# AtharvRN/dflash

Hardware: AMD Instinct MI355X
Metric: accepted_tokens_per_sec (higher is better)
Workload: dtype bf16

## Files before the change

### dflash_amd/csrc/attn_head.hip

```cpp
#include "gemm_rows.h"
#include <stdlib.h>
#include <type_traits>

namespace {

typedef __attribute__((address_space(3))) bf16x4 lds_bf16x4;

struct HeadAttnArgs {
  const bf16_t *xq;
  int64_t ldq;
  int q_col, k_col, v_col;
  const bf16_t *xc;
  int64_t ldc;
  int ck_col, cv_col;
  const bf16_t *q_w, *k_w;
  float eps;
  const bf16_t *cos_tab, *sin_tab;
  int max_pos;
  bf16_t *kc, *vc;
  int cache_rows;
  int n_q, n_kv, G;
  float scale_log2;
  int causal;
  const int32_t *dyn;
  int S, tau, bs, pos0;
  bf16x8 *out_frag;
  int64_t out_tile_stride;
  float *o_part;
  float *ml_part;
  int *tickets;
  int ns_old;
  int64_t xq_cand_stride, out_cand_stride, ws_cand_stride, cache_cand_stride;
  int dyn_cand_stride;
  const float *xq32;
  int64_t part_stride32;
  int nparts32;
  bf16_t *k_out, *v_out;
  int64_t kv_out_cand_stride;
  int out_rows;
};

__device__ __forceinline__ void swap16(float &a, float &b) {
  asm volatile("s_nop 1\n\tv_permlane16_swap_b32 %0, %1" : "+v"(a), "+v"(b));
}
__device__ __forceinline__ void swap32(float &a, float &b) {
  asm volatile("s_nop 1\n\tv_permlane32_swap_b32 %0, %1" : "+v"(a), "+v"(b));
}
__device__ __forceinline__ float wave_g_max(float v) {
  float a = v, b = v;
  swap16(a, b);
  a = b = fmaxf(a, b);
  swap32(a, b);
  return fmaxf(a, b);
}
__device__ __forceinline__ float wave_g_sum(float v) {
  float a = v, b = v;
  swap16(a, b);
  a = b = a + b;
  swap32(a, b);
  return a + b;
}

template <int NP>
struct RopeLoads {
  bf16x8 xv[NP], cs[NP], sn[NP], wv;
  f32x4 pa[NP][2], pb[NP][2];
};

template <int NP>
__device__ __forceinline__ void rope_issue(const bf16_t *const (&src)[NP], const int (&pos)[NP], const bf16_t *nw,
                                           const bf16_t *cos_tab, const bf16_t *sin_tab, int max_pos, const bf16_t *safe,
                                           int l, RopeLoads<NP> &ld) {
  const int d0 = (l & 15) * 8;
#pragma unroll
  for (int p = 0; p < NP; ++p) {
    ld.xv[p] = *reinterpret_cast<const bf16x8 *>((src[p] ? src[p] : safe) + d0);
    int pp = pos[p] < max_pos ? pos[p] : max_pos - 1;
    pp = pp < 0 ? 0 : pp;
    ld.cs[p] = *reinterpret_cast<const bf16x8 *>(cos_tab + (int64_t)pp * 64 + (d0 & 63));
    ld.sn[p] = *reinterpret_cast<const bf16x8 *>(sin_tab + (int64_t)pp * 64 + (d0 & 63));
  }
  ld.wv = *reinterpret_cast<const bf16x8 *>((nw ? nw : safe) + d0);
}

template <int NP>
__device__ __forceinline__ void rope_issue32(const float *const (&src)[NP], const int (&pos)[NP], const bf16_t *nw,
                                             const bf16_t *cos_tab, const bf16_t *sin_tab, int max_pos, const float *safe32,
                                             const bf16_t *safe, int64_t part_stride, int nparts, int l, RopeLoads<NP> &ld) {
  const int d0 = (l & 15) * 8;
  const int64_t ps = nparts > 1 ? part_stride : 0;
#pragma unroll
  for (int p = 0; p < NP; ++p) {
    const float *b = (src[p] ? src[p] : safe32) + d0;
    ld.pa[p][0] = *reinterpret_cast<const f32x4 *>(b);
    ld.pa[p][1] = *reinterpret_cast<const f32x4 *>(b + 4);
    ld.pb[p][0] = *reinterpret_cast<const f32x4 *>(b + ps);
    ld.pb[p][1] = *reinterpret_cast<const f32x4 *>(b + ps + 4);
    int pp = pos[p] < max_pos ? pos[p] : max_pos - 1;
    pp = pp < 0 ? 0 : pp;
    ld.cs[p] = *reinterpret_cast<const bf16x8 *>(cos_tab + (int64_t)pp * 64 + (d0 & 63));
    ld.sn[p] = *reinterpret_cast<const bf16x8 *>(sin_tab + (int64_t)pp * 64 + (d0 & 63));
  }
  ld.wv = *reinterpret_cast<const bf16x8 *>((nw ? nw : safe) + d0);
}
template <int NP>
__device__ __forceinline__ void rope_sum32(RopeLoads<NP> &ld, int nparts) {
#pragma unroll
  for (int p = 0; p < NP; ++p)
#pragma unroll
    for (int j = 0; j < 8; ++j) {
      const float s0 = ld.pa[p][j >> 2][j & 3], s1 = ld.pb[p][j >> 2][j & 3];
      ld.xv[p][j] = f2bf(nparts > 1 ? s0 + s1 : s0);
    }
}

template <int NP>
__device__ __forceinline__ void rope_finish(const RopeLoads<NP> &ld, const bool (&rope)[NP], bool has_norm, float eps, int l,
                                            bf16x8 (&out)[NP]) {
  const int c = l & 15;
#pragma unroll
  for (int p = 0; p < NP; ++p) {
    float x[8], n[8];
    float ss = 0.f;
#pragma unroll
    for (int j = 0; j < 8; ++j) {
      x[j] = bf2f(ld.xv[p][j]);
      ss += x[j] * x[j];
    }
    if (has_norm) {
      ss += __builtin_bit_cast(float, __builtin_amdgcn_mov_dpp(__builtin_bit_cast(int, ss), 0xB1, 0xF, 0xF, true));
      ss += __builtin_bit_cast(float, __builtin_amdgcn_mov_dpp(__builtin_bit_cast(int, ss), 0x4E, 0xF, 0xF, true));
      ss += __builtin_bit_cast(float, __builtin_amdgcn_mov_dpp(__builtin_bit_cast(int, ss), 0x141, 0xF, 0xF, true));
      ss += __builtin_bit_cast(float, __builtin_amdgcn_mov_dpp(__builtin_bit_cast(int, ss), 0x140, 0xF, 0xF, true));
      const float rstd = rsqrtf(ss * (1.f / 128.f) + eps);
#pragma unroll
      for (int j = 0; j < 8; ++j) n[j] = rbf(bf2f(ld.wv[j]) * rbf(x[j] * rstd));
    } else {
#pragma unroll
      for (int j = 0; j < 8; ++j) n[j] = x[j];
    }
#pragma unroll
    for (int j = 0; j < 8; ++j) {
      const float pn =
          __builtin_bit_cast(float, __builtin_amdgcn_mov_dpp(__builtin_bit_cast(int, n[j]), 0x128, 0xF, 0xF, true));
      const float cj = bf2f(ld.cs[p][j]), sj = bf2f(ld.sn[p][j]);
      const float r = rbf(rbf(n[j] * cj) + rbf((c < 8 ? -pn : pn) * sj));
      out[p][j] = f2bf(rope[p] ? r : x[j]);
    }
  }
}

template <int NP>
__device__ __forceinline__ void rope_items(const bf16_t *const (&src)[NP], const int (&pos)[NP], const bool (&rope)[NP],
                                           const bf16_t *nw, float eps, const bf16_t *cos_tab, const bf16_t *sin_tab,
                                           int max_pos, const bf16_t *safe, int l, bf16x8 (&out)[NP]) {
  RopeLoads<NP> ld;
  rope_issue<NP>(src, pos, nw, cos_tab, sin_tab, max_pos, safe, l, ld);
  rope_finish<NP>(ld, rope, nw != nullptr, eps, l, out);
}

__device__ __forceinline__ int k_swz(int row, int ch) { return row * 256 + ((ch ^ (row & 15)) << 4); }
__device__ __forceinline__ int v_swz(int row, int ch) {
  return row * 256 + ((((ch >> 1) ^ (row & 7)) << 5) | ((ch & 1) << 4));
}

#ifdef DFL_ATTN_STAMPS
__device__ unsigned long long g_hstamps[2][8];
#define HSTAMP(i)                                                                                  \
  do {                                                                                             \
    if (tid == 0 && kvh == 0 && hh == 0 && (split == 0 || is_new))                                 \
      g_hstamps[is_new ? 1 : 0][i] = __builtin_amdgcn_s_memrealtime();                             \
  } while (0)
__device__ unsigned long long g_ostamps[2][8];
__device__ unsigned long long g_amax[16];
#define OSTAMP(i)                                                                                  \
  do {                                                                                             \
    if (tid == 0 && (t == 0 || t == p.ntiles - 1)) g_ostamps[t ? 1 : 0][i] = __builtin_amdgcn_s_memrealtime(); \
  } while (0)
#else
#define HSTAMP(i)
#define OSTAMP(i)
#endif

template <int QT, int NW>
struct HeadLds {
  static_assert(NW * 4 >= QT * 16 && NW * 8192 >= 32768, "q rows: 4 per wave; new K / V: two 32-row tiles each");
  static constexpr int kVPriv = NW * 8192;
  static constexpr int kQ = kVPriv;
  static constexpr int kLoop = kVPriv + QT * 4096;
  static constexpr int kRow = 132;
  static constexpr int kMergeO = 0;
  static constexpr int kMergeML = NW * QT * 16 * kRow * 4;
  static constexpr int kMerge = kMergeML + NW * QT * 128;
  static constexpr int kRaw = kLoop > kMerge ? kLoop : kMerge;
  static constexpr int kBytes = NW < 8 ? kRaw : (kRaw > 84 * 1024 ? kRaw : 84 * 1024);
};

template <int QT, int NW, bool SIGNAL, bool HP = false, bool XF32 = false>
__device__ __forceinline__ void attn_head_body(const HeadAttnArgs &a, char *lds, int *s_last_p, const int kvh, const int by,
                                               const int cand, int *done_ctr) {
  static_assert(!HP || QT == 2, "head pairs use the two-tile register layout");
  using L = HeadLds<QT, NW>;
  int &s_last = *s_last_p;

  const int tid = threadIdx.x;
  const int w = __builtin_amdgcn_readfirstlane(tid >> 6), l = tid & 63;
  const int hpg = HP ? a.G >> 1 : a.G;
  const int hh = by % hpg, split = by / hpg;
  const int head = kvh * a.G + (HP ? 2 * hh : hh);
  const int ns = a.ns_old + 1;
  const bool is_new = split == a.ns_old;
  int S = a.S, tau = a.tau, bs = a.bs, pos0 = a.pos0;
  if (a.dyn) {
    const int32_t *dp = a.dyn + cand * a.dyn_cand_stride;
    S = dp[DFL_DYN_S];
    tau = dp[DFL_DYN_TAU];
    bs = dp[DFL_DYN_BS];
    pos0 = dp[DFL_DYN_POS0];
  }
  const int n_new = tau + bs;
  const int qi = l & 15, g = l >> 4;
  HSTAMP(0);
  const bf16_t *const xq = XF32 ? a.cos_tab : a.xq + cand * a.xq_cand_stride;
  const float *const xq32 = XF32 ? a.xq32 + cand * a.xq_cand_stride : nullptr;
  bf16x8 *const out_frag = a.out_frag + cand * a.out_cand_stride;
  float *const o_part = a.o_part + cand * a.ws_cand_stride;
  float *const ml_part = a.ml_part + cand * a.ws_cand_stride;
  int *const tickets = a.tickets + cand * a.ws_cand_stride;
  bf16_t *const kc = a.kc + cand * a.cache_cand_stride, *const vc = a.vc + cand * a.cache_cand_stride;
  bf16_t *const k_new = a.k_out ? a.k_out + cand * a.kv_out_cand_stride : kc;
  bf16_t *const v_new = a.k_out ? a.v_out + cand * a.kv_out_cand_stride : vc;
  const int new_rows_cap = a.k_out ? a.out_rows : a.cache_rows;
  const int new_row0 = a.k_out ? 0 : S;
  const bf16_t *kbase = kc + (int64_t)kvh * a.cache_rows * 128;
  const bf16_t *vbase = vc + (int64_t)kvh * a.cache_rows * 128;


  int t0 = 0, t1 = 0;
  if (!is_new && a.ns_old > 0) {
    const int nt = (S + 31) >> 5;
    const int tps = (nt + a.ns_old - 1) / a.ns_old;
    t0 = split * tps;
    t1 = t0 + tps;
    t0 = t0 > nt ? nt : t0;
    t1 = t1 > nt ? nt : t1;
  }
  const int old_last = S > 0 ? S - 1 : 0;
  bf16x8 kA[2][4], vA[8], kB[2][4], vB[8];
  auto fetch_k = [&](bf16x8(&kf)[2][4], int t, int lim) {
#pragma unroll
    for (int u = 0; u < 2; ++u) {
      int row = t * 32 + u * 16 + qi;
      row = row < lim ? row : lim;
#pragma unroll
      for (int s = 0; s < 4; ++s)
        kf[u][s] = *reinterpret_cast<const bf16x8 *>(kbase + (int64_t)row * 128 + s * 32 + g * 8);
    }
  };
  auto fetch_v = [&](bf16x8(&vr)[8], int t, int lim) {
#pragma unroll
    for (int i = 0; i < 8; ++i) {
      const int c = l + 64 * i;
      int row = t * 32 + (c >> 4);
      row = row < lim ? row : lim;
      vr[i] = *reinterpret_cast<const bf16x8 *>(vbase + (int64_t)row * 128 + (c & 15) * 8);
    }
  };
  auto fetch = [&](bf16x8(&kf)[2][4], bf16x8(&vr)[8], int t, int lim) {
    fetch_k(kf, t, lim);
    fetch_v(vr, t, lim);
  };
  char *q_lds = lds + L::kQ;
  const int jq = 4 * w + g;
  const int jrow = HP ? jq & 15 : jq;
  const int jhead = HP ? head + (jq >> 4) : head;
  RopeLoads<1> qld;
  {
    const int pos[1] = {pos0 + tau + jrow};
    if constexpr (XF32) {
      const float *src[1] = {jrow < bs ? xq32 + (int64_t)jrow * a.ldq + a.q_col + jhead * 128 : nullptr};
      rope_issue32<1>(src, pos, a.q_w, a.cos_tab, a.sin_tab, a.max_pos, xq32, xq, a.part_stride32, a.nparts32, l, qld);
    } else {
      const bf16_t *src[1] = {jrow < bs ? xq + (int64_t)jrow * a.ldq + a.q_col + jhead * 128 : nullptr};
      rope_issue<1>(src, pos, a.q_w, a.cos_tab, a.sin_tab, a.max_pos, xq, l, qld);
    }
  }
  asm volatile("" ::: "memory");
  auto finish_q = [&]() {
    if (jq < QT * 16) {
      const bool rp[1] = {true};
      bf16x8 ov[1];
      if constexpr (XF32) rope_sum32<1>(qld, a.nparts32);
      rope_finish<1>(qld, rp, a.q_w != nullptr, a.eps, l, ov);
      const bf16x8 z = {0, 0, 0, 0, 0, 0, 0, 0};
      *reinterpret_cast<bf16x8 *>(q_lds + (jq >> 4) * 4096 + k_swz(jq & 15, qi)) = jrow < bs ? ov[0] : z;
    }
  };
  int tcur = t0 + w;
  char *new_k = lds, *new_v = lds + 16384;
  if (!is_new) {
    fetch(kA, vA, tcur < t1 ? tcur : 0, old_last);
    asm volatile("" ::: "memory");
    finish_q();
  } else {
    auto sweep = [&](auto np_tag) {
      constexpr int NP = decltype(np_tag)::value;
      const bf16_t *src[NP];
      const float *src32[NP];
      int pos[NP], rel[NP];
      bool rp[NP], isv[NP];
      bf16x8 ov[NP];
#pragma unroll
      for (int p = 0; p < NP; ++p) {
        const int it = (p * NW + w) * 4 + g;
        isv[p] = it >= n_new;
        rel[p] = isv[p] ? it - n_new : it;
        const bool ok = it < 2 * n_new;
        const int vsel = isv[p] ? 1 : 0;
        if constexpr (XF32) {
          src32[p] = ok ? xq32 + (int64_t)rel[p] * a.ldq + a.k_col + vsel * (a.v_col - a.k_col) + kvh * 128 : nullptr;
          src[p] = ok ? xq : nullptr;
        } else {
          const bf16_t *row = rel[p] < tau ? a.xc + (int64_t)rel[p] * a.ldc + a.ck_col + vsel * (a.cv_col - a.ck_col)
                                           : xq + (int64_t)(rel[p] - tau) * a.ldq + a.k_col + vsel * (a.v_col - a.k_col);
          src[p] = ok ? row + kvh * 128 : nullptr;
          src32[p] = nullptr;
        }
        pos[p] = pos0 + rel[p];
        rp[p] = !isv[p];
      }
      RopeLoads<NP> kld;
      if constexpr (XF32)
        rope_issue32<NP>(src32, pos, a.k_w, a.cos_tab, a.sin_tab, a.max_pos, xq32, xq, a.part_stride32, a.nparts32, l, kld);
      else
        rope_issue<NP>(src, pos, a.k_w, a.cos_tab, a.sin_tab, a.max_pos, xq, l, kld);
      asm volatile("" ::: "memory");
      finish_q();
      if constexpr (XF32) rope_sum32<NP>(kld, a.nparts32);
      rope_finish<NP>(kld, rp, a.k_w != nullptr, a.eps, l, ov);
#pragma unroll
      for (int p = 0; p < NP; ++p)
        if (src[p]) {
          const int jt = rel[p] >> 5, r = rel[p] & 31;
          *reinterpret_cast<bf16x8 *>((isv[p] ? new_v + jt * 8192 + v_swz(r, qi) : new_k + jt * 8192 + k_swz(r, qi))) = ov[p];
          const int crow = new_row0 + rel[p];
          if (hh == 0 && crow < new_rows_cap)
            *reinterpret_cast<bf16x8 *>((isv[p] ? v_new : k_new) + ((int64_t)kvh * new_rows_cap + crow) * 128 + qi * 8) = ov[p];
        }
    };
    if (2 * n_new <= NW * 4)
      sweep(std::integral_constant<int, 1>{});
    else if (2 * n_new <= NW * 8)
      sweep(std::integral_constant<int, 2>{});
    else
      sweep(std::integral_constant<int, 4>{});
  }
  HSTAMP(1);
  __syncthreads();

  bf16x8 qf[QT][4];
#pragma unroll
  for (int qt = 0; qt < QT; ++qt)
#pragma unroll
    for (int s = 0; s < 4; ++s) qf[qt][s] = *reinterpret_cast<const bf16x8 *>(q_lds + qt * 4096 + k_swz(qi, s * 4 + g));

  f32x4 o[QT][8];
  float m_run[QT], l_run[QT];
#pragma unroll
  for (int qt = 0; qt < QT; ++qt) {
    m_run[qt] = -INFINITY;
    l_run[qt] = 0.f;
#pragma unroll
    for (int dt = 0; dt < 8; ++dt) o[qt][dt] = (f32x4){0.f, 0.f, 0.f, 0.f};
  }

  auto compute = [&](const bf16x8(&kf)[2][4], const char *vt, int key0, int nvalid, int vrows, bool new_rows) {
    const int qq = qi >> 2, p4 = l & 3;
    int r0 = 4 * g + qq, r1 = 16 + 4 * g + qq;
    r0 = r0 < vrows ? r0 : vrows - 1;
    r1 = r1 < vrows ? r1 : vrows - 1;
#pragma unroll
    for (int qt = 0; qt < QT; ++qt) {
      f32x4 sc[2];
#pragma unroll
      for (int u = 0; u < 2; ++u) {
        sc[u] = (f32x4){0.f, 0.f, 0.f, 0.f};
#pragma unroll
        for (int s = 0; s < 4; ++s) sc[u] = __builtin_amdgcn_mfma_f32_16x16x32_bf16(kf[u][s], qf[qt][s], sc[u], 0, 0, 0);
      }
      float mx = -INFINITY;
#pragma unroll
      for (int u = 0; u < 2; ++u)
#pragma unroll
        for (int r = 0; r < 4; ++r) {
          const int key = key0 + u * 16 + 4 * g + r;
          const bool vis = key < nvalid && (!new_rows || !a.causal || key <= tau + (HP ? 0 : qt * 16) + qi);
          const float v = vis ? sc[u][r] * a.scale_log2 : -INFINITY;
          sc[u][r] = v;
          mx = fmaxf(mx, v);
        }
      mx = wave_g_max(mx);
      const float m_new = fmaxf(m_run[qt], mx);
      const float m_ref = m_new == -INFINITY ? 0.f : m_new;
      const float alpha = __builtin_amdgcn_exp2f(m_run[qt] - m_ref);
      m_run[qt] = m_new;
      float psum = 0.f;
      bf16x8 pb;
#pragma unroll
      for (int u = 0; u < 2; ++u)
#pragma unroll
        for (int r = 0; r < 4; ++r) {
          const float p = __builtin_amdgcn_exp2f(sc[u][r] - m_ref);
          psum += p;
          pb[u * 4 + r] = f2bf(p);
        }
      l_run[qt] = l_run[qt] * alpha + psum;
#pragma unroll
      for (int dt = 0; dt < 8; ++dt) o[qt][dt] *= alpha;
#pragma unroll
      for (int dt = 0; dt < 8; ++dt) {
        const bf16x4 v0 =
            __builtin_amdgcn_ds_read_tr16_b64_v4bf16((lds_bf16x4 *)(vt + r0 * 256 + (((dt ^ (r0 & 7)) << 5) | (p4 << 3))));
        const bf16x4 v1 =
            __builtin_amdgcn_ds_read_tr16_b64_v4bf16((lds_bf16x4 *)(vt + r1 * 256 + (((dt ^ (r1 & 7)) << 5) | (p4 << 3))));
        const bf16x8 va = {v0[0], v0[1], v0[2], v0[3], v1[0], v1[1], v1[2], v1[3]};
        o[qt][dt] = __builtin_amdgcn_mfma_f32_16x16x32_bf16(va, pb, o[qt][dt], 0, 0, 0);
      }
    }
  };

  if (is_new) {
    const int ntile = (n_new + 31) >> 5;
    if (w < ntile) {
      bf16x8 kf[2][4];
#pragma unroll
      for (int u = 0; u < 2; ++u)
#pragma unroll
        for (int s = 0; s < 4; ++s)
          kf[u][s] = *reinterpret_cast<const bf16x8 *>(new_k + w * 8192 + k_swz(u * 16 + qi, s * 4 + g));
      int vrows = n_new - w * 32;
      vrows = vrows > 32 ? 32 : vrows;
      compute(kf, new_v + w * 8192, w * 32, n_new, vrows, true);
    }
  } else {
    char *my_v = lds + w * 8192;
    auto put_v = [&](const bf16x8(&vr)[8]) {
#pragma unroll
      for (int i = 0; i < 8; ++i) {
        const int c = l + 64 * i;
        *reinterpret_cast<bf16x8 *>(my_v + v_swz(c >> 4, c & 15)) = vr[i];
      }
    };
    if (tcur + NW >= t1) {
      if (tcur < t1) {
        put_v(vA);
        compute(kA, my_v, tcur * 32, S, 32, false);
      }
    } else if (QT == 1) {
      for (; tcur < t1; tcur += 2 * NW) {
        fetch(kB, vB, tcur + NW, tcur + NW < t1 ? old_last : 0);
        put_v(vA);
        compute(kA, my_v, tcur * 32, S, 32, false);
        fetch(kA, vA, tcur + 2 * NW, tcur + 2 * NW < t1 ? old_last : 0);
        if (tcur + NW < t1) {
          put_v(vB);
          compute(kB, my_v, (tcur + NW) * 32, S, 32, false);
        }
      }
    } else {
      for (; tcur < t1; tcur += NW) {
        const int lim = tcur + NW < t1 ? old_last : 0;
        put_v(vA);
        fetch_v(vA, tcur + NW, lim);
        compute(kA, my_v, tcur * 32, S, 32, false);
        fetch_k(kA, tcur + NW, lim);
      }
    }
  }

  HSTAMP(2);
  __syncthreads();
  HSTAMP(3);
  {
    float *mo = reinterpret_cast<float *>(lds + L::kMergeO);
    float *mml = reinterpret_cast<float *>(lds + L::kMergeML);
#pragma unroll
    for (int qt = 0; qt < QT; ++qt) {
      const float lt = wave_g_sum(l_run[qt]);
      float *op = mo + ((w * QT + qt) * 16 + qi) * L::kRow;
#pragma unroll
      for (int dt = 0; dt < 8; ++dt) *reinterpret_cast<f32x4 *>(op + dt * 16 + 4 * g) = o[qt][dt];
      if (g == 0) {
        mml[((w * QT + qt) * 16 + qi) * 2] = m_run[qt];
        mml[((w * QT + qt) * 16 + qi) * 2 + 1] = lt;
      }
    }
  }
  __syncthreads();
  const bool has_item = tid < QT * 256;
  const int qt = tid >> 8, q = (tid >> 4) & 15, dg = tid & 15;
  float M = -INFINITY, Lsum = 0.f, acc[8];
#pragma unroll
  for (int j = 0; j < 8; ++j) acc[j] = 0.f;
  if (has_item) {
    const float *mo = reinterpret_cast<const float *>(lds + L::kMergeO);
    const float *mml = reinterpret_cast<const float *>(lds + L::kMergeML);
    float ms[NW], ls[NW];
#pragma unroll
    for (int ww = 0; ww < NW; ++ww) {
      ms[ww] = mml[((ww * QT + qt) * 16 + q) * 2];
      ls[ww] = mml[((ww * QT + qt) * 16 + q) * 2 + 1];
      M = fmaxf(M, ms[ww]);
    }
    const float mref = M == -INFINITY ? 0.f : M;
#pragma unroll
    for (int ww = 0; ww < NW; ++ww) {
      const float wgt = __builtin_amdgcn_exp2f(ms[ww] - mref);
      const float *op = mo + ((ww * QT + qt) * 16 + q) * L::kRow + dg * 8;
      const f32x4 a0 = *reinterpret_cast<const f32x4 *>(op), a1 = *reinterpret_cast<const f32x4 *>(op + 4);
      Lsum += wgt * ls[ww];
#pragma unroll
      for (int j = 0; j < 4; ++j) {
        acc[j] += wgt * a0[j];
        acc[4 + j] += wgt * a1[j];
      }
    }
  }
  auto emit = [&](float Lt, const float(&v)[8]) {
    const float inv = Lt > 0.f ? 1.f / Lt : 0.f;
    bf16x8 r;
#pragma unroll
    for (int j = 0; j < 8; ++j) r[j] = f2bf(v[j] * inv);
    if (SIGNAL && q >= bs) r = (bf16x8){0, 0, 0, 0, 0, 0, 0, 0};
    bf16x8 *dst = HP ? &out_frag[((head + qt) * 16 + dg) * 16 + q] : &out_frag[qt * a.out_tile_stride + (head * 16 + dg) * 16 + q];
    if (SIGNAL) {
      const __amdgpu_buffer_rsrc_t rd = __builtin_amdgcn_make_buffer_rsrc(dst, 0, 16, 0x00020000);
      __builtin_amdgcn_raw_buffer_store_b128(__builtin_bit_cast(u32x4, r), rd, 0, 0, 16);
    } else {
      *dst = r;
    }
  };
  auto signal = [&]() {
    if (SIGNAL) {
      asm volatile("s_waitcnt vmcnt(0)" ::: "memory");
      __syncthreads();
      if (tid < 32) __hip_atomic_fetch_add(done_ctr + tid * 32, 1, __ATOMIC_RELAXED, __HIP_MEMORY_SCOPE_AGENT);
#ifdef DFL_ATTN_STAMPS
      if (tid == 0) atomicMax(&g_amax[15], (unsigned long long)__builtin_amdgcn_s_memrealtime());
#endif
    }
  };
  HSTAMP(4);
  if (ns == 1) {
    if (has_item) emit(Lsum, acc);
    signal();
    return;
  }

  const size_t item_row = HP ? (size_t)(head + qt) * 16 + q : (size_t)head * (QT * 16) + qt * 16 + q;
  const size_t rows_per_split = (size_t)a.n_q * (HP ? 16 : QT * 16);
  const __amdgpu_buffer_rsrc_t ro =
      __builtin_amdgcn_make_buffer_rsrc(o_part, 0, (int)(rows_per_split * ns * 128 * sizeof(float)), 0x00020000);
  const __amdgpu_buffer_rsrc_t rm =
      __builtin_amdgcn_make_buffer_rsrc(ml_part, 0, (int)(rows_per_split * ns * 2 * sizeof(float)), 0x00020000);
  if (has_item) {
    const int off = (int)((((size_t)split * rows_per_split + item_row) * 128 + dg * 8) * sizeof(float));
    const f32x4 s0 = {acc[0], acc[1], acc[2], acc[3]}, s1 = {acc[4], acc[5], acc[6], acc[7]};
    __builtin_amdgcn_raw_buffer_store_b128(__builtin_bit_cast(u32x4, s0), ro, off, 0, 16);
    __builtin_amdgcn_raw_buffer_store_b128(__builtin_bit_cast(u32x4, s1), ro, off + 16, 0, 16);
    if (dg == 0) {
      const int offm = (int)((((size_t)split * rows_per_split + item_row) * 2) * sizeof(float));
      __builtin_amdgcn_raw_buffer_store_b32(__builtin_bit_cast(unsigned, M), rm, offm, 0, 16);
      __builtin_amdgcn_raw_buffer_store_b32(__builtin_bit_cast(unsigned, Lsum), rm, offm + 4, 0, 16);
    }
  }
  asm volatile("s_waitcnt vmcnt(0)" ::: "memory");
  __syncthreads();
  HSTAMP(5);
  if (tid == 0) {
    const int ticket = __hip_atomic_fetch_add(&tickets[head], 1, __ATOMIC_RELAXED, __HIP_MEMORY_SCOPE_AGENT);
    const int last = ticket == ns - 1;
    if (last) __hip_atomic_store(&tickets[head], 0, __ATOMIC_RELAXED, __HIP_MEMORY_SCOPE_AGENT);
    s_last = last;
  }
  __syncthreads();
  HSTAMP(6);
#ifdef DFL_ATTN_STAMPS
  if (tid == 0) atomicMax(&g_amax[split < 15 ? split : 14], (unsigned long long)__builtin_amdgcn_s_memrealtime());
#endif
  if (!s_last) return;

  if (has_item) {
    float Mg = -INFINITY, Lg = 0.f, ag[8];
#pragma unroll
    for (int j = 0; j < 8; ++j) ag[j] = 0.f;
    constexpr int U = 8;
    for (int s = 0; s < ns; s += U) {
      float ms[U], ls[U];
      f32x4 a0[U], a1[U];
#pragma unroll
      for (int u = 0; u < U; ++u) {
        const int sc = s + u < ns ? s + u : ns - 1;
        const int off = (int)((((size_t)sc * rows_per_split + item_row) * 128 + dg * 8) * sizeof(float));
        const int offm = (int)((((size_t)sc * rows_per_split + item_row) * 2) * sizeof(float));
        ms[u] = __builtin_bit_cast(float, __builtin_amdgcn_raw_buffer_load_b32(rm, offm, 0, 16));
        ls[u] = __builtin_bit_cast(float, __builtin_amdgcn_raw_buffer_load_b32(rm, offm + 4, 0, 16));
        a0[u] = __builtin_bit_cast(f32x4, __builtin_amdgcn_raw_buffer_load_b128(ro, off, 0, 16));
        a1[u] = __builtin_bit_cast(f32x4, __builtin_amdgcn_raw_buffer_load_b128(ro, off + 16, 0, 16));
      }
      float mnew = Mg;
#pragma unroll
      for (int u = 0; u < U; ++u) mnew = fmaxf(mnew, s + u < ns ? ms[u] : -INFINITY);
      const float mref = mnew == -INFINITY ? 0.f : mnew;
      const float scale = __builtin_amdgcn_exp2f(Mg - mref);
      Mg = mnew;
      Lg *= scale;
#pragma unroll
      for (int j = 0; j < 8; ++j) ag[j] *= scale;
#pragma unroll
      for (int u = 0; u < U; ++u) {
        const float wgt = s + u < ns ? __builtin_amdgcn_exp2f(ms[u] - mref) : 0.f;
        Lg += wgt * ls[u];
#pragma unroll
        for (int j = 0; j < 4; ++j) {
          ag[j] += wgt * a0[u][j];
          ag[4 + j] += wgt * a1[u][j];
        }
      }
    }
    emit(Lg, ag);
  }
  signal();
#ifdef DFL_ATTN_STAMPS
  asm volatile("s_waitcnt vmcnt(0)" ::: "memory");
#endif
  HSTAMP(7);
}

template <int QT>
__global__ __launch_bounds__(512) void k_attn_head(HeadAttnArgs a) {
  __shared__ __attribute__((aligned(16))) char lds[HeadLds<QT, 8>::kBytes];
  __shared__ int s_last;
  attn_head_body<QT, 8, false>(a, lds, &s_last, blockIdx.x, blockIdx.y, blockIdx.z, nullptr);
}

__global__ __launch_bounds__(512) void k_attn_head_pair(HeadAttnArgs a) {
  __shared__ __attribute__((aligned(16))) char lds[HeadLds<2, 8>::kBytes];
  __shared__ int s_last;
  attn_head_body<2, 8, false, true>(a, lds, &s_last, blockIdx.x, blockIdx.y, blockIdx.z, nullptr);
}

__global__ __launch_bounds__(512) void k_attn_head32(HeadAttnArgs a) {
  __shared__ __attribute__((aligned(16))) char lds[HeadLds<1, 8>::kBytes];
  __shared__ int s_last;
  attn_head_body<1, 8, false, false, true>(a, lds, &s_last, blockIdx.x, blockIdx.y, blockIdx.z, nullptr);
}
__global__ __launch_bounds__(512) void k_attn_head_pair32(HeadAttnArgs a) {
  __shared__ __attribute__((aligned(16))) char lds[HeadLds<2, 8>::kBytes];
  __shared__ int s_last;
  attn_head_body<2, 8, false, true, true>(a, lds, &s_last, blockIdx.x, blockIdx.y, blockIdx.z, nullptr);
}

struct AttnOArgs {
  HeadAttnArgs at;
  int n_attn;
  const bf16x8 *wo;
  int KS, ntiles;
  bf16_t *h_io;
  int64_t ldh;
  float *ss_out;
  int *done;
  int *o_done, *fail;
  int done_target;
};

__global__ __launch_bounds__(256, 2) void k_attn_oproj(AttnOArgs p) {
  __shared__ __attribute__((aligned(16))) char lds[HeadLds<1, 4>::kBytes];
  __shared__ int s_last;
  const int b = blockIdx.x;
  if (b < p.n_attn) {
    attn_head_body<1, 4, true>(p.at, lds, &s_last, b % p.at.n_kv, b / p.at.n_kv, 0, p.done);
    return;
  }
  const int t = b - p.n_attn;
  const int tid = threadIdx.x;
  const int w = __builtin_amdgcn_readfirstlane(tid >> 6), l = tid & 63;
  OSTAMP(0);
  bf16x8 wv[4][8];
  {
    const bf16x8 *base = p.wo + ((size_t)t * p.KS + 32 * w) * 64;
#pragma unroll
    for (int c = 0; c < 4; ++c) {
      int nf = p.KS - 32 * w - 8 * c;
      nf = nf < 0 ? 0 : (nf > 8 ? 8 : nf);
      load_ksteps<8>(wv[c], base + c * 8 * 64, nf, l);
    }
  }
#ifdef DFL_ATTN_STAMPS
  OSTAMP(1);
  asm volatile("s_waitcnt vmcnt(0)" ::: "memory");
  OSTAMP(2);
#endif
  if (tid == 0) {
    const unsigned long long t0 = __builtin_amdgcn_s_memrealtime();
    const int *mine = p.done + (t & 31) * 32;
    while (__hip_atomic_load(mine, __ATOMIC_RELAXED, __HIP_MEMORY_SCOPE_AGENT) < p.done_target) {
      __builtin_amdgcn_s_sleep(8);
      if (__builtin_amdgcn_s_memrealtime() - t0 > 200000ull) {
        *p.fail = 1;
        break;
      }
    }
  }
  OSTAMP(3);
  __syncthreads();
  f32x4 acc = {0.f, 0.f, 0.f, 0.f};
  {
    const __amdgpu_buffer_rsrc_t rx =
        __builtin_amdgcn_make_buffer_rsrc(const_cast<bf16x8 *>(p.at.out_frag), 0, p.KS * 1024, 0x00020000);
#pragma unroll
    for (int c = 0; c < 4; ++c) {
      bf16x8 xv[8];
#pragma unroll
      for (int f = 0; f < 8; ++f)
        xv[f] = __builtin_bit_cast(bf16x8, __builtin_amdgcn_raw_buffer_load_b128(rx, ((32 * w + 8 * c + f) * 64 + l) * 16, 0, 16));
#pragma unroll
      for (int f = 0; f < 8; ++f) acc = __builtin_amdgcn_mfma_f32_16x16x32_bf16(wv[c][f], xv[f], acc, 0, 0, 0);
    }
  }
  float *red = reinterpret_cast<float *>(lds);
  *reinterpret_cast<f32x4 *>(&red[w * 256 + l * 4]) = acc;
  OSTAMP(4);
  __syncthreads();
  OSTAMP(5);
  {
    const int m = tid >> 4, nl = tid & 15;
    const int idx = 4 * (m + 16 * (nl >> 2)) + (nl & 3);
    float s = 0.f;
#pragma unroll
    for (int ww = 0; ww < 4; ++ww) s += red[ww * 256 + idx];
    const int n = t * 16 + nl;
    const float v = rbf(s);
    bf16_t *hp = p.h_io + (int64_t)m * p.ldh + n;
    const float hn = rbf(bf2f(*hp) + v);
    *hp = f2bf(hn);
    const float qs = row_sum16(hn * hn);
    if (nl == 0 && p.ss_out) p.ss_out[t * 16 + m] = qs;
  }
#ifdef DFL_ATTN_STAMPS
  asm volatile("s_waitcnt vmcnt(0)" ::: "memory");
#endif
  OSTAMP(6);
  if (tid == 0) {
    const int k = __hip_atomic_fetch_add(p.o_done, 1, __ATOMIC_RELAXED, __HIP_MEMORY_SCOPE_AGENT);
    if (k == p.ntiles - 1) {
      for (int r = 0; r < 32; ++r) __hip_atomic_store(p.done + r * 32, 0, __ATOMIC_RELAXED, __HIP_MEMORY_SCOPE_AGENT);
      __hip_atomic_store(p.o_done, 0, __ATOMIC_RELAXED, __HIP_MEMORY_SCOPE_AGENT);
    }
  }
}

}

#ifdef DFL_ATTN_STAMPS
extern "C" int dfl_debug_read_head_stamps(unsigned long long *host_out) {
  return (int)hipMemcpyFromSymbol(host_out, HIP_SYMBOL(g_hstamps), sizeof(unsigned long long) * 16);
}
extern "C" int dfl_debug_read_attn_max(unsigned long long *host_out) {
  const int rc = (int)hipMemcpyFromSymbol(host_out, HIP_SYMBOL(g_amax), sizeof(unsigned long long) * 16);
  unsigned long long z[16] = {};
  return rc ? rc : (int)hipMemcpyToSymbol(HIP_SYMBOL(g_amax), z, sizeof(z));
}
extern "C" int dfl_debug_read_oproj_stamps(unsigned long long *host_out) {
  return (int)hipMemcpyFromSymbol(host_out, HIP_SYMBOL(g_ostamps), sizeof(unsigned long long) * 16);
}
#endif

extern "C" int64_t dfl_attn_head_ws_bytes(int n_q, int max_splits, int q_tiles) {
  const int64_t b = (int64_t)max_splits * n_q * q_tiles * 16 * (128 + 2) * sizeof(float) + (int64_t)n_q * sizeof(int) + 64;
  return (b + 15) / 16 * 16;
}

namespace {
bool pair_ok_forced(int knob, bool has_tail, int q_tiles, int G, int bs) {
  return knob == 1 && !has_tail && q_tiles == 1 && G % 2 == 0 && bs <= 16;
}

struct OprojTail {
  const void *wo;
  int q_dim, H;
  void *h_io;
  int64_t ldh;
  float *ss_out;
  int32_t *sync;
};

int attn_head_launch(const void *xq, int64_t ldq, int q_col, int k_col, int v_col, const void *xc, int64_t ldc, int ck_col,
                     int cv_col, int n_q, int n_kv, const void *q_norm_w, const void *k_norm_w, float eps,
                     const void *cos_tab, const void *sin_tab, int max_pos, void *kcache, void *vcache, int cache_rows,
                     float scale, int causal, const int32_t *dyn, int S, int tau, int bs, int pos0, int q_tiles, void *ws,
                     int max_splits, void *out_frag, int64_t out_tile_stride, int n_cand, int64_t xq_cand_stride,
                     int64_t out_cand_stride, void *k_out, void *v_out, int64_t kv_out_cand_stride, int out_rows,
                     int dyn_cand_stride, int64_t cache_cand_stride, void *stream, const OprojTail *tail = nullptr,
                     int nparts32 = 0, int64_t part_stride32 = 0) {
  DFL_REQUIRE(xq && cos_tab && sin_tab && kcache && vcache && out_frag && ws, "dfl_attn_head: null pointer");
  DFL_REQUIRE(nparts32 >= 0 && nparts32 <= 2 && (nparts32 == 0 || (!tail && q_tiles == 1 && tau == 0 && !xc && part_stride32 % 4 == 0)),
              "dfl_attn_head: the fp32-partials form takes 1 or 2 K parts, one query tile, no context rows");
  DFL_REQUIRE((q_norm_w == nullptr) == (k_norm_w == nullptr), "dfl_attn_head: give both norm weights or neither");
  DFL_REQUIRE(n_q > 0 && n_kv > 0 && n_q % n_kv == 0, "dfl_attn_head: bad head counts (n_q=%d n_kv=%d)", n_q, n_kv);
  DFL_REQUIRE(q_tiles == 1 || q_tiles == 2, "dfl_attn_head: q_tiles must be 1 or 2");
  DFL_REQUIRE(ldq > 0 && ldq % 8 == 0 && q_col >= 0 && k_col >= 0 && v_col >= 0 && q_col % 8 == 0 && k_col % 8 == 0 &&
                  v_col % 8 == 0 && max_pos > 0,
              "dfl_attn_head: bad block-row layout");
  DFL_REQUIRE(S >= 0 && tau >= 0 && tau <= 32 && bs >= 1 && bs <= 16 * q_tiles && tau + bs <= 64,
              "dfl_attn_head: lengths S=%d tau=%d bs=%d outside the kernel's range (q_tiles=%d)", S, tau, bs, q_tiles);
  DFL_REQUIRE(tau == 0 || (xc && ldc > 0 && ldc % 8 == 0 && ck_col >= 0 && cv_col >= 0 && ck_col % 8 == 0 && cv_col % 8 == 0),
              "dfl_attn_head: context rows without a context source");
  DFL_REQUIRE(S + (k_out ? 0 : tau + bs) <= cache_rows, "dfl_attn_head: S + tau + bs = %d exceeds cache_rows = %d", S + tau + bs,
              cache_rows);
  DFL_REQUIRE(max_splits >= 1 && out_tile_stride >= 0 && out_tile_stride % 8 == 0, "dfl_attn_head: bad max_splits / out_tile_stride");
  DFL_REQUIRE(n_cand >= 1 && n_cand <= 64, "dfl_attn_head: n_cand outside 1..64");
  DFL_REQUIRE(n_cand == 1 || (xq_cand_stride % 8 == 0 && out_cand_stride % 8 == 0 && cache_cand_stride % 8 == 0 &&
                              ((k_out && v_out) || cache_cand_stride >= (int64_t)n_kv * cache_rows * 128)),
              "dfl_attn_head: several blocks per launch need 8-element strides and either a K/V staging area "
              "(candidates on one cache) or a cache per request");
  DFL_REQUIRE(!k_out == !v_out && (!k_out || (out_rows >= tau + bs && kv_out_cand_stride >= (int64_t)n_kv * out_rows * 128)),
              "dfl_attn_head: bad K/V staging area");
  const int G = n_q / n_kv;
  const int nt = (S + 31) / 32;
  static const int knob_tiles = [] { const char *e = getenv("DFL_ATTN_HEAD_TILES"); return e ? atoi(e) : 8; }();
  static const int knob_wgs = [] { const char *e = getenv("DFL_ATTN_HEAD_WGS"); return e ? atoi(e) : 224; }();
  static const int knob_wgsm = [] { const char *e = getenv("DFL_ATTN_HEAD_WGS_MULTI"); return e ? atoi(e) : 256; }();
  static const int knob_wgs4 = [] { const char *e = getenv("DFL_ATTN_OPROJ_WGS"); return e ? atoi(e) : 256; }();
  static const int knob_tiles4 = [] { const char *e = getenv("DFL_ATTN_OPROJ_TILES"); return e ? atoi(e) : 4; }();
  const int tiles = tail ? (knob_tiles4 < 1 ? 1 : knob_tiles4) : (knob_tiles < 1 ? 1 : knob_tiles);
  int ns_old = (nt + tiles - 1) / tiles;
  int budget = (tail ? knob_wgs4 : (n_cand > 1 ? knob_wgsm : knob_wgs)) / (n_q * n_cand) - 1;
  budget = budget < 1 ? 1 : budget;
  ns_old = ns_old > budget ? budget : ns_old;
  static const int knob_pair = [] { const char *e = getenv("DFL_ATTN_HEAD_PAIR"); return e ? atoi(e) : -1; }();
  bool pair = !tail && q_tiles == 1 && G % 2 == 0 && bs <= 16 && nt > tiles * ns_old && (nt > 160 || n_cand > 2);
  if (knob_pair >= 0) pair = pair_ok_forced(knob_pair, tail != nullptr, q_tiles, G, bs);
  if (pair) {
    int budget2 = (n_cand > 1 ? knob_wgsm : knob_wgs) / ((n_q / 2) * n_cand) - 1;
    budget2 = budget2 < 1 ? 1 : budget2;
    ns_old = (nt + tiles - 1) / tiles;
    ns_old = ns_old > budget2 ? budget2 : ns_old;
  }
  ns_old = ns_old > max_splits - 1 ? max_splits - 1 : ns_old;
  if (nt == 0 && !dyn) ns_old = 0;
  HeadAttnArgs a{};
  a.xq = (const bf16_t *)xq;
  a.ldq = ldq;
  a.q_col = q_col;
  a.k_col = k_col;
  a.v_col = v_col;
  a.xc = (const bf16_t *)xc;
  a.ldc = ldc;
  a.ck_col = ck_col;
  a.cv_col = cv_col;
  a.q_w = (const bf16_t *)q_norm_w;
  a.k_w = (const bf16_t *)k_norm_w;
  a.eps = eps;
  a.cos_tab = (const bf16_t *)cos_tab;
  a.sin_tab = (const bf16_t *)sin_tab;
  a.max_pos = max_pos;
  a.kc = (bf16_t *)kcache;
  a.vc = (bf16_t *)vcache;
  a.cache_rows = cache_rows;
  a.n_q = n_q;
  a.n_kv = n_kv;
  a.G = G;
  a.scale_log2 = scale * 1.4426950408889634f;
  a.causal = causal ? 1 : 0;
  a.dyn = dyn;
  a.S = S;
  a.tau = tau;
  a.bs = bs;
  a.pos0 = pos0;
  a.out_frag = (bf16x8 *)out_frag;
  a.out_tile_stride = out_tile_stride / 8;
  const int64_t rows = (int64_t)max_splits * n_q * q_tiles * 16;
  a.o_part = (float *)ws;
  a.ml_part = (float *)ws + rows * 128;
  a.tickets = (int *)((float *)ws + rows * 130);
  a.ns_old = ns_old;
  a.xq_cand_stride = xq_cand_stride;
  a.out_cand_stride = out_cand_stride / 8;
  a.ws_cand_stride = dfl_attn_head_ws_bytes(n_q, max_splits, q_tiles) / 4;
  a.k_out = (bf16_t *)k_out;
  a.v_out = (bf16_t *)v_out;
  a.kv_out_cand_stride = kv_out_cand_stride;
  a.out_rows = out_rows;
  a.dyn_cand_stride = dyn_cand_stride;
  a.cache_cand_stride = cache_cand_stride;
  const dim3 grid(n_kv, (pair ? G / 2 : G) * (ns_old + 1), n_cand);
  hipStream_t st = (hipStream_t)stream;
  if (nparts32 > 0) {
    a.xq = nullptr;
    a.xq32 = (const float *)xq;
    a.nparts32 = nparts32;
    a.part_stride32 = part_stride32;
    if (pair)
      hipLaunchKernelGGL(k_attn_head_pair32, grid, dim3(512), 0, st, a);
    else
      hipLaunchKernelGGL(k_attn_head32, grid, dim3(512), 0, st, a);
    DFL_CHECK_LAUNCH("dfl_attn_head_batch_f32");
    return DFL_OK;
  }
  if (pair) {
    hipLaunchKernelGGL(k_attn_head_pair, grid, dim3(512), 0, st, a);
    DFL_CHECK_LAUNCH("dfl_attn_head");
    return DFL_OK;
  }
  if (tail) {
    AttnOArgs p{};
    p.at = a;
    p.n_attn = n_kv * G * (ns_old + 1);
    p.wo = (const bf16x8 *)tail->wo;
    p.KS = tail->q_dim / 32;
    p.ntiles = tail->H / 16;
    p.h_io = (bf16_t *)tail->h_io;
    p.ldh = tail->ldh;
    p.ss_out = tail->ss_out;
    p.done = tail->sync;
    p.o_done = tail->sync + 1024;
    p.fail = tail->sync + 1025;
    p.done_target = n_q;
    hipLaunchKernelGGL(k_attn_oproj, dim3(p.n_attn + p.ntiles), dim3(256), 0, st, p);
    DFL_CHECK_LAUNCH("dfl_attn_head_oproj");
    return DFL_OK;
  }
  if (q_tiles == 1)
    hipLaunchKernelGGL(k_attn_head<1>, grid, dim3(512), 0, st, a);
  else
    hipLaunchKernelGGL(k_attn_head<2>, grid, dim3(512), 0, st, a);
  DFL_CHECK_LAUNCH("dfl_attn_head");
  return DFL_OK;
}
}

extern "C" int dfl_attn_head(const void *xq, int64_t ldq, int q_col, int k_col, int v_col, const void *xc, int64_t ldc,
                             int ck_col, int cv_col, int n_q, int n_kv, const void *q_norm_w, const void *k_norm_w,
                             float eps, const void *cos_tab, const void *sin_tab, int max_pos, void *kcache,
                             void *vcache, int cache_rows, float scale, int causal, const int32_t *dyn, int S, int tau,
                             int bs, int pos0, int q_tiles, void *ws, int max_splits, void *out_frag,
                             int64_t out_tile_stride, void *stream) {
  return attn_head_launch(xq, ldq, q_col, k_col, v_col, xc, ldc, ck_col, cv_col, n_q, n_kv, q_norm_w, k_norm_w, eps, cos_tab,
                          sin_tab, max_pos, kcache, vcache, cache_rows, scale, causal, dyn, S, tau, bs, pos0, q_tiles, ws,
                          max_splits, out_frag, out_tile_stride, 1, 0, 0, nullptr, nullptr, 0, 0, 0, 0, stream);
}

extern "C" int dfl_attn_head_oproj(const void *xq, int64_t ldq, int q_col, int k_col, int v_col, const void *xc, int64_t ldc,
                                   int ck_col, int cv_col, int n_q, int n_kv, const void *q_norm_w, const void *k_norm_w,
                                   float eps, const void *cos_tab, const void *sin_tab, int max_pos, void *kcache,
                                   void *vcache, int cache_rows, float scale, int causal, const int32_t *dyn, int S, int tau,
                                   int bs, int pos0, void *ws, int max_splits, void *attn_frag, const void *wo_packed, int H,
                                   void *h_io, int64_t ldh, float *ss_out, int32_t *sync, void *stream) {
  DFL_REQUIRE(wo_packed && h_io && sync, "dfl_attn_head_oproj: null pointer");
  DFL_REQUIRE(H > 0 && H % 16 == 0 && ldh >= H && n_q * 128 <= 4096 && bs <= 16 && tau + bs <= 32,
              "dfl_attn_head_oproj: H=%d q_dim=%d tau=%d bs=%d outside the kernel's range (q_dim <= 4096, tau + bs <= 32)", H,
              n_q * 128, tau, bs);
  const OprojTail tail{wo_packed, n_q * 128, H, h_io, ldh, ss_out, sync};
  return attn_head_launch(xq, ldq, q_col, k_col, v_col, xc, ldc, ck_col, cv_col, n_q, n_kv, q_norm_w, k_norm_w, eps, cos_tab,
                          sin_tab, max_pos, kcache, vcache, cache_rows, scale, causal, dyn, S, tau, bs, pos0, 1, ws, max_splits,
                          attn_frag, 0, 1, 0, 0, nullptr, nullptr, 0, 0, 0, 0, stream, &tail);
}

extern "C" int dfl_attn_head_cand(const void *xq, int64_t ldq, int q_col, int k_col, int v_col, int n_cand,
                                  int64_t xq_cand_stride, int n_q, int n_kv, const void *q_norm_w, const void *k_norm_w,
                                  float eps, const void *cos_tab, const void *sin_tab, int max_pos, const void *kcache,
                                  const void *vcache, int cache_rows, float scale, int S, int bs, void *ws, int max_splits,
                                  void *out_frag, int64_t out_cand_stride, void *k_out, void *v_out,
                                  int64_t kv_out_cand_stride, int out_rows, void *stream) {
  DFL_REQUIRE(n_cand >= 1 && k_out && v_out, "dfl_attn_head_cand: needs the K/V staging area");
  return attn_head_launch(xq, ldq, q_col, k_col, v_col, nullptr, 0, 0, 0, n_q, n_kv, q_norm_w, k_norm_w, eps, cos_tab, sin_tab,
                          max_pos, const_cast<void *>(kcache), const_cast<void *>(vcache), cache_rows, scale, 1, nullptr, S, 0,
                          bs, S, 1, ws, max_splits, out_frag, 0, n_cand, xq_cand_stride, out_cand_stride, k_out, v_out,
                          kv_out_cand_stride, out_rows, 0, 0, stream);
}

extern "C" int dfl_attn_head_batch(const void *xq, int64_t ldq, int q_col, int k_col, int v_col, int R, int64_t xq_req_stride,
                                   int n_q, int n_kv, const void *q_norm_w, const void *k_norm_w, float eps,
                                   const void *cos_tab, const void *sin_tab, int max_pos, void *kcache, void *vcache,
                                   int cache_rows, int64_t cache_req_stride, float scale, int causal, const int32_t *dyn,
                                   int kv_len_max, void *ws, int max_splits, void *out_frag, int64_t out_req_stride,
                                   void *stream) {
  DFL_REQUIRE(dyn, "dfl_attn_head_batch: the requests' lengths come from dyn (R records)");
  DFL_REQUIRE(kv_len_max >= 16 && kv_len_max <= cache_rows, "dfl_attn_head_batch: kv_len_max=%d outside 16..cache_rows", kv_len_max);
  return attn_head_launch(xq, ldq, q_col, k_col, v_col, nullptr, 0, 0, 0, n_q, n_kv, q_norm_w, k_norm_w, eps, cos_tab, sin_tab,
                          max_pos, kcache, vcache, cache_rows, scale, causal, dyn, kv_len_max - 16, 0, 16, 0, 1, ws, max_splits,
                          out_frag, 0, R, xq_req_stride, out_req_stride, nullptr, nullptr, 0, 0, DFL_DYN_WORDS, cache_req_stride,
                          stream);
}

extern "C" int dfl_attn_head_batch_t(const void *xq, int64_t ldq, int q_col, int k_col, int v_col, int R, int64_t xq_req_stride,
                                     int n_q, int n_kv, const void *q_norm_w, const void *k_norm_w, float eps,
                                     const void *cos_tab, const void *sin_tab, int max_pos, void *kcache, void *vcache,
                                     int cache_rows, int64_t cache_req_stride, float scale, int causal, const int32_t *dyn,
                                     int kv_len_max, void *ws, int max_splits, void *out_frag, int64_t out_req_stride,
                                     int64_t out_tile_stride, int q_tiles, void *stream) {
  DFL_REQUIRE(dyn, "dfl_attn_head_batch_t: the requests' lengths come from dyn (R records)");
  DFL_REQUIRE(q_tiles == 1 || q_tiles == 2, "dfl_attn_head_batch_t: q_tiles must be 1 or 2");
  DFL_REQUIRE(kv_len_max >= 16 * q_tiles && kv_len_max <= cache_rows, "dfl_attn_head_batch_t: kv_len_max=%d outside range", kv_len_max);
  return attn_head_launch(xq, ldq, q_col, k_col, v_col, nullptr, 0, 0, 0, n_q, n_kv, q_norm_w, k_norm_w, eps, cos_tab, sin_tab,
                          max_pos, kcache, vcache, cache_rows, scale, causal, dyn, kv_len_max - 16 * q_tiles, 0, 16 * q_tiles, 0,
                          q_tiles, ws, max_splits, out_frag, out_tile_stride, R, xq_req_stride, out_req_stride, nullptr, nullptr, 0,
                          0, DFL_DYN_WORDS, cache_req_stride, stream);
}

extern "C" int dfl_attn_head_cand_t(const void *xq, int64_t ldq, int q_col, int k_col, int v_col, int n_cand,
                                    int64_t xq_cand_stride, int n_q, int n_kv, const void *q_norm_w, const void *k_norm_w,
                                    float eps, const void *cos_tab, const void *sin_tab, int max_pos, const void *kcache,
                                    const void *vcache, int cache_rows, float scale, int S, int bs, void *ws, int max_splits,
                                    void *out_frag, int64_t out_cand_stride, int64_t out_tile_stride, int q_tiles, void *k_out,
                                    void *v_out, int64_t kv_out_cand_stride, int out_rows, void *stream) {
  DFL_REQUIRE(n_cand >= 1 && k_out && v_out, "dfl_attn_head_cand_t: needs the K/V staging area");
  DFL_REQUIRE(q_tiles == 1 || q_tiles == 2, "dfl_attn_head_cand_t: q_tiles must be 1 or 2");
  return attn_head_launch(xq, ldq, q_col, k_col, v_col, nullptr, 0, 0, 0, n_q, n_kv, q_norm_w, k_norm_w, eps, cos_tab, sin_tab,
                          max_pos, const_cast<void *>(kcache), const_cast<void *>(vcache), cache_rows, scale, 1, nullptr, S, 0,
                          bs, S, q_tiles, ws, max_splits, out_frag, out_tile_stride, n_cand, xq_cand_stride, out_cand_stride, k_out,
                          v_out, kv_out_cand_stride, out_rows, 0, 0, stream);
}

extern "C" int dfl_attn_head_batch_f32(const float *xq_parts, int nparts, int64_t part_stride, int64_t ldq, int q_col, int k_col,
                                       int v_col, int R, int64_t xq_req_stride, int n_q, int n_kv, const void *q_norm_w,
                                       const void *k_norm_w, float eps, const void *cos_tab, const void *sin_tab, int max_pos,
                                       void *kcache, void *vcache, int cache_rows, int64_t cache_req_stride, float scale,
                                       int causal, const int32_t *dyn, int kv_len_max, void *ws, int max_splits,
                                       void *out_frag, int64_t out_req_stride, void *stream) {
  DFL_REQUIRE(dyn, "dfl_attn_head_batch_f32: the requests' lengths come from dyn (R records)");
  DFL_REQUIRE(nparts == 1 || nparts == 2, "dfl_attn_head_batch_f32: 1 or 2 K parts (got %d)", nparts);
  DFL_REQUIRE(kv_len_max >= 16 && kv_len_max <= cache_rows, "dfl_attn_head_batch_f32: kv_len_max=%d outside 16..cache_rows",
              kv_len_max);
  return attn_head_launch(xq_parts, ldq, q_col, k_col, v_col, nullptr, 0, 0, 0, n_q, n_kv, q_norm_w, k_norm_w, eps, cos_tab,
                          sin_tab, max_pos, kcache, vcache, cache_rows, scale, causal, dyn, kv_len_max - 16, 0, 16, 0, 1, ws,
                          max_splits, out_frag, 0, R, xq_req_stride, out_req_stride, nullptr, nullptr, 0, 0, DFL_DYN_WORDS,
                          cache_req_stride, stream, nullptr, nparts, part_stride);
}
```

Before: 1740.

## Hand off split-merge per wave and preload packed head kernel arguments

```diff
diff --git a/dflash_amd/csrc/attn_head.hip b/dflash_amd/csrc/attn_head.hip
--- a/dflash_amd/csrc/attn_head.hip
+++ b/dflash_amd/csrc/attn_head.hip
@@ -40,6 +40,77 @@
   int out_rows;
 };
 
+struct AttnHeadBits {
+  uint64_t G : 7, ns_old : 9, causal : 1, nparts32 : 2, q_col8 : 15, k_col8 : 15, v_col8 : 15;
+};
+static_assert(sizeof(AttnHeadBits) == 8, "AttnHeadBits is one 64-bit kernel argument");
+struct AttnHead {
+  const int32_t *dyn;
+  bf16_t *kc, *vc;
+  const void *xq;
+  uint64_t bits;
+  int dyn_cand_stride, cache_rows, ldq, max_pos;
+};
+#define ATTN_HEAD_DWORDS 14
+static_assert(sizeof(AttnHead) == 4 * ATTN_HEAD_DWORDS, "the head is what the hardware preloads: at most 14 dwords, no padding");
+#define ATTN_HEAD_PARAMS \
+  const int32_t *dyn, bf16_t *kc, bf16_t *vc, const void *xq, uint64_t bits, int dyn_cand_stride, int cache_rows, int ldq, int max_pos
+#define ATTN_HEAD_NAMES dyn, kc, vc, xq, bits, dyn_cand_stride, cache_rows, ldq, max_pos
+#define ATTN_HEAD_OF(h) (h).dyn, (h).kc, (h).vc, (h).xq, (h).bits, (h).dyn_cand_stride, (h).cache_rows, (h).ldq, (h).max_pos
+
+template <bool XF32>
+__device__ __forceinline__ HeadAttnArgs with_head(HeadAttnArgs a, ATTN_HEAD_PARAMS) {
+  const AttnHeadBits b = __builtin_bit_cast(AttnHeadBits, bits);
+  a.dyn = dyn;
+  a.dyn_cand_stride = dyn_cand_stride;
+  a.kc = kc;
+  a.vc = vc;
+  if (XF32)
+    a.xq32 = reinterpret_cast<const float *>(xq);
+  else
+    a.xq = reinterpret_cast<const bf16_t *>(xq);
+  a.cache_rows = cache_rows;
+  a.ldq = ldq;
+  a.max_pos = max_pos;
+  a.G = (int)b.G;
+  a.ns_old = (int)b.ns_old;
+  a.causal = (int)b.causal;
+  if (XF32) a.nparts32 = (int)b.nparts32;
+  a.q_col = (int)b.q_col8 * 8;
+  a.k_col = (int)b.k_col8 * 8;
+  a.v_col = (int)b.v_col8 * 8;
+  return a;
+}
+
+bool attn_head_head(AttnHead &h, const HeadAttnArgs &a) {
+  AttnHeadBits b{};
+  b.G = a.G;
+  b.ns_old = a.ns_old;
+  b.causal = a.causal;
+  b.nparts32 = a.nparts32;
+  b.q_col8 = a.q_col / 8;
+  b.k_col8 = a.k_col / 8;
+  b.v_col8 = a.v_col / 8;
+  const bool fits = (int)b.G == a.G && (int)b.ns_old == a.ns_old && (int)b.causal == a.causal && (int)b.nparts32 == a.nparts32 &&
+                    (int)b.q_col8 * 8 == a.q_col && (int)b.k_col8 * 8 == a.k_col && (int)b.v_col8 * 8 == a.v_col &&
+                    a.ldq == (int)a.ldq;
+  if (!fits) {
+    dfl_set_error("dfl_attn_head: launch arguments outside the preloaded head's fields (G=%d, splits %d, columns %d/%d/%d, ldq=%lld)",
+                  a.G, a.ns_old + 1, a.q_col, a.k_col, a.v_col, (long long)a.ldq);
+    return false;
+  }
+  h.dyn = a.dyn;
+  h.kc = a.kc;
+  h.vc = a.vc;
+  h.xq = a.nparts32 > 0 ? (const void *)a.xq32 : (const void *)a.xq;
+  h.bits = __builtin_bit_cast(uint64_t, b);
+  h.dyn_cand_stride = a.dyn_cand_stride;
+  h.cache_rows = a.cache_rows;
+  h.ldq = (int)a.ldq;
+  h.max_pos = a.max_pos;
+  return true;
+}
+
 __device__ __forceinline__ void swap16(float &a, float &b) {
   asm volatile("s_nop 1\n\tv_permlane16_swap_b32 %0, %1" : "+v"(a), "+v"(b));
 }
@@ -201,7 +272,6 @@
                                                const int cand, int *done_ctr) {
   static_assert(!HP || QT == 2, "head pairs use the two-tile register layout");
   using L = HeadLds<QT, NW>;
-  int &s_last = *s_last_p;
 
   const int tid = threadIdx.x;
   const int w = __builtin_amdgcn_readfirstlane(tid >> 6), l = tid & 63;
@@ -557,6 +627,8 @@
     return;
   }
 
+  constexpr bool kWaveHandoff = !SIGNAL;
+  if (kWaveHandoff && !has_item) return;
   const size_t item_row = HP ? (size_t)(head + qt) * 16 + q : (size_t)head * (QT * 16) + qt * 16 + q;
   const size_t rows_per_split = (size_t)a.n_q * (HP ? 16 : QT * 16);
   const __amdgpu_buffer_rsrc_t ro =
@@ -575,20 +647,39 @@
     }
   }
   asm volatile("s_waitcnt vmcnt(0)" ::: "memory");
-  __syncthreads();
-  HSTAMP(5);
-  if (tid == 0) {
-    const int ticket = __hip_atomic_fetch_add(&tickets[head], 1, __ATOMIC_RELAXED, __HIP_MEMORY_SCOPE_AGENT);
-    const int last = ticket == ns - 1;
-    if (last) __hip_atomic_store(&tickets[head], 0, __ATOMIC_RELAXED, __HIP_MEMORY_SCOPE_AGENT);
-    s_last = last;
-  }
-  __syncthreads();
-  HSTAMP(6);
+  if constexpr (kWaveHandoff) {
+    HSTAMP(5);
+    int last = 0;
+    if (l == 0) {
+      int *const tk = &tickets[head * (QT * 4) + w];
+      const int ticket = __hip_atomic_fetch_add(tk, 1, __ATOMIC_RELAXED, __HIP_MEMORY_SCOPE_AGENT);
+      last = ticket == ns - 1;
+      if (last) __hip_atomic_store(tk, 0, __ATOMIC_RELAXED, __HIP_MEMORY_SCOPE_AGENT);
+    }
+    last = __builtin_amdgcn_readfirstlane(last);
+    asm volatile("" ::: "memory");
+    HSTAMP(6);
 #ifdef DFL_ATTN_STAMPS
-  if (tid == 0) atomicMax(&g_amax[split < 15 ? split : 14], (unsigned long long)__builtin_amdgcn_s_memrealtime());
+    if (tid == 0) atomicMax(&g_amax[split < 15 ? split : 14], (unsigned long long)__builtin_amdgcn_s_memrealtime());
 #endif
-  if (!s_last) return;
+    if (!last) return;
+  } else {
+    int &s_last = *s_last_p;
+    __syncthreads();
+    HSTAMP(5);
+    if (tid == 0) {
+      const int ticket = __hip_atomic_fetch_add(&tickets[head], 1, __ATOMIC_RELAXED, __HIP_MEMORY_SCOPE_AGENT);
+      const int last = ticket == ns - 1;
+      if (last) __hip_atomic_store(&tickets[head], 0, __ATOMIC_RELAXED, __HIP_MEMORY_SCOPE_AGENT);
+      s_last = last;
+    }
+    __syncthreads();
+    HSTAMP(6);
+#ifdef DFL_ATTN_STAMPS
+    if (tid == 0) atomicMax(&g_amax[split < 15 ? split : 14], (unsigned long long)__builtin_amdgcn_s_memrealtime());
+#endif
+    if (!s_last) return;
+  }
 
   if (has_item) {
     float Mg = -INFINITY, Lg = 0.f, ag[8];
@@ -637,28 +728,26 @@
   HSTAMP(7);
 }
 
+#define ATTN_KERNEL_PARAMS ATTN_HEAD_PARAMS, HeadAttnArgs rest
+#define ATTN_KERNEL_ARGS(XF32) with_head<XF32>(rest, ATTN_HEAD_NAMES)
 template <int QT>
-__global__ __launch_bounds__(512) void k_attn_head(HeadAttnArgs a) {
+__global__ __launch_bounds__(512) void k_attn_head(ATTN_KERNEL_PARAMS) {
   __shared__ __attribute__((aligned(16))) char lds[HeadLds<QT, 8>::kBytes];
-  __shared__ int s_last;
-  attn_head_body<QT, 8, false>(a, lds, &s_last, blockIdx.x, blockIdx.y, blockIdx.z, nullptr);
-}
-
-__global__ __launch_bounds__(512) void k_attn_head_pair(HeadAttnArgs a) {
+  attn_head_body<QT, 8, false>(ATTN_KERNEL_ARGS(false), lds, nullptr, blockIdx.x, blockIdx.y, blockIdx.z, nullptr);
+}
+
+__global__ __launch_bounds__(512) void k_attn_head_pair(ATTN_KERNEL_PARAMS) {
   __shared__ __attribute__((aligned(16))) char lds[HeadLds<2, 8>::kBytes];
-  __shared__ int s_last;
-  attn_head_body<2, 8, false, true>(a, lds, &s_last, blockIdx.x, blockIdx.y, blockIdx.z, nullptr);
-}
-
-__global__ __launch_bounds__(512) void k_attn_head32(HeadAttnArgs a) {
+  attn_head_body<2, 8, false, true>(ATTN_KERNEL_ARGS(false), lds, nullptr, blockIdx.x, blockIdx.y, blockIdx.z, nullptr);
+}
+
+__global__ __launch_bounds__(512) void k_attn_head32(ATTN_KERNEL_PARAMS) {
   __shared__ __attribute__((aligned(16))) char lds[HeadLds<1, 8>::kBytes];
-  __shared__ int s_last;
-  attn_head_body<1, 8, false, false, true>(a, lds, &s_last, blockIdx.x, blockIdx.y, blockIdx.z, nullptr);
-}
-__global__ __launch_bounds__(512) void k_attn_head_pair32(HeadAttnArgs a) {
+  attn_head_body<1, 8, false, false, true>(ATTN_KERNEL_ARGS(true), lds, nullptr, blockIdx.x, blockIdx.y, blockIdx.z, nullptr);
+}
+__global__ __launch_bounds__(512) void k_attn_head_pair32(ATTN_KERNEL_PARAMS) {
   __shared__ __attribute__((aligned(16))) char lds[HeadLds<2, 8>::kBytes];
-  __shared__ int s_last;
-  attn_head_body<2, 8, false, true, true>(a, lds, &s_last, blockIdx.x, blockIdx.y, blockIdx.z, nullptr);
+  attn_head_body<2, 8, false, true, true>(ATTN_KERNEL_ARGS(true), lds, nullptr, blockIdx.x, blockIdx.y, blockIdx.z, nullptr);
 }
 
 struct AttnOArgs {
@@ -777,7 +866,7 @@
 #endif
 
 extern "C" int64_t dfl_attn_head_ws_bytes(int n_q, int max_splits, int q_tiles) {
-  const int64_t b = (int64_t)max_splits * n_q * q_tiles * 16 * (128 + 2) * sizeof(float) + (int64_t)n_q * sizeof(int) + 64;
+  const int64_t b = (int64_t)max_splits * n_q * q_tiles * 16 * (128 + 2) * sizeof(float) + (int64_t)n_q * 8 * sizeof(int) + 64;
   return (b + 15) / 16 * 16;
 }
 
@@ -896,20 +985,24 @@
   a.cache_cand_stride = cache_cand_stride;
   const dim3 grid(n_kv, (pair ? G / 2 : G) * (ns_old + 1), n_cand);
   hipStream_t st = (hipStream_t)stream;
+#define ATTN_LAUNCH_ARGS ATTN_HEAD_OF(h), a
+  AttnHead h{};
   if (nparts32 > 0) {
     a.xq = nullptr;
     a.xq32 = (const float *)xq;
     a.nparts32 = nparts32;
     a.part_stride32 = part_stride32;
+    if (!attn_head_head(h, a)) return DFL_EINVAL;
     if (pair)
-      hipLaunchKernelGGL(k_attn_head_pair32, grid, dim3(512), 0, st, a);
+      hipLaunchKernelGGL(k_attn_head_pair32, grid, dim3(512), 0, st, ATTN_LAUNCH_ARGS);
     else
-      hipLaunchKernelGGL(k_attn_head32, grid, dim3(512), 0, st, a);
+      hipLaunchKernelGGL(k_attn_head32, grid, dim3(512), 0, st, ATTN_LAUNCH_ARGS);
     DFL_CHECK_LAUNCH("dfl_attn_head_batch_f32");
     return DFL_OK;
   }
+  if (!tail && !attn_head_head(h, a)) return DFL_EINVAL;
   if (pair) {
-    hipLaunchKernelGGL(k_attn_head_pair, grid, dim3(512), 0, st, a);
+    hipLaunchKernelGGL(k_attn_head_pair, grid, dim3(512), 0, st, ATTN_LAUNCH_ARGS);
     DFL_CHECK_LAUNCH("dfl_attn_head");
     return DFL_OK;
   }
@@ -932,9 +1025,9 @@
     return DFL_OK;
   }
   if (q_tiles == 1)
-    hipLaunchKernelGGL(k_attn_head<1>, grid, dim3(512), 0, st, a);
+    hipLaunchKernelGGL(k_attn_head<1>, grid, dim3(512), 0, st, ATTN_LAUNCH_ARGS);
   else
-    hipLaunchKernelGGL(k_attn_head<2>, grid, dim3(512), 0, st, a);
+    hipLaunchKernelGGL(k_attn_head<2>, grid, dim3(512), 0, st, ATTN_LAUNCH_ARGS);
   DFL_CHECK_LAUNCH("dfl_attn_head");
   return DFL_OK;
 }
```

Result: no change. 1726 (-0.8%).
